# zrudnick/bramble

Hardware: AMD Instinct MI355X
Metric: projected alignments/sec vs GENCODE-scale annotation (higher is better)
Workload: dtype u32; 1 GPU; device-resident (inputs already in HBM, packed rows left in HBM): 10M paired-end 2x100 short reads (name-collated, unstranded) vs GENCODE-shaped synthetic annotation (250836 transcripts, 1684128 transcript-exon rows, 25 refs); BASELINE.json configs[1]; group_lanes=8, seed=0xb4a3b1e

## Files before the change

### bramble_amd/csrc/direct_kernels.inc

```

#define WAVE_SYNC()                                                \
  do {                                                             \
    __builtin_amdgcn_fence(__ATOMIC_RELEASE, "workgroup");         \
    __builtin_amdgcn_wave_barrier();                               \
    __builtin_amdgcn_fence(__ATOMIC_ACQUIRE, "workgroup");         \
  } while (0)

__global__ void __launch_bounds__(256) k_name_seed(DirectArgs D) {
  const int64_t g = (int64_t)blockIdx.x * blockDim.x + threadIdx.x;
  if (g >= D.n_groups) return;
  const uint32_t a0 = D.group_off[g];
  const uint32_t no = D.name_off[a0];
  Mt64Lazy gen;
  gen.seed(hash_bytes(D.names + no, D.name_off[a0 + 1] - no));
  D.rnd0[g] = gen();
}
__device__ __forceinline__ uint32_t pick_from(uint64_t z0, const uint8_t *name, uint64_t len, uint32_t n) {
  uint64_t hi, lo;
  mul64wide(z0, (uint64_t)n, hi, lo);
  if (lo < (uint64_t)n) {
    const uint64_t thr = (0 - (uint64_t)n) % (uint64_t)n;
    if (lo < thr) return primary_pick(name, len, n);
  }
  return (uint32_t)hi;
// ... 586 lines not shown
#pragma unroll
      for (int st = 32; st; st >>= 1) if (sh_pre[wv][l + st] <= e) l += st;
      D.m_aln[first + e] = sh_v[wv][l];
    }
  }
}

template <int CLS>
__global__ void __launch_bounds__(256, CLS == 1 ? 8 : 6) k_emit_rows(ProjectArgs A, DirectArgs D, int64_t first, int64_t n_end) {
  __shared__ uint32_t sh_cig[CLS == 1 ? 1 : 256 * LDS_SLOT];
  __shared__ uint16_t sh_mops[CLS == 1 ? 1 : 256];
  if (CLS != 1) {
    sh_mops[threadIdx.x] = (uint16_t)((merge_action(threadIdx.x >> 4, threadIdx.x & 15u) << 8) | merge_ops(threadIdx.x >> 4, threadIdx.x & 15u));
    __syncthreads();
  }
  const int64_t e64 = first + (int64_t)blockIdx.x * blockDim.x + threadIdx.x;
  if (e64 >= n_end) return;
  const DevIndex &ix = A.ix;
  const DevCfg &cfg = A.cfg;
  typedef uint32_t ntl4 __attribute__((ext_vector_type(4)));
  typedef uint32_t ntl2 __attribute__((ext_vector_type(2)));
  const uint32_t a = __builtin_nontemporal_load(D.m_aln + e64);
  if (a == 0xffffffffu) return;
  const ntl4 hd_ = __builtin_nontemporal_load((const ntl4 *)(A.head + a)), rg_ = __builtin_nontemporal_load((const ntl4 *)(A.ranges + a));
  const ntl2 f_ = __builtin_nontemporal_load((const ntl2 *)(D.fm + a)), gd_ = __builtin_nontemporal_load((const ntl2 *)(D.gd + a)), dp_ = __builtin_nontemporal_load((const ntl2 *)(D.dpos + a));
  const uint4 hd = make_uint4(hd_.x, hd_.y, hd_.z, hd_.w), rg = make_uint4(rg_.x, rg_.y, rg_.z, rg_.w);
  const uint2 f = make_uint2(f_.x, f_.y), gd = make_uint2(gd_.x, gd_.y), dp = make_uint2(dp_.x, dp_.y);
  const uint4 E = make_uint4(gd.x, gd.y, dp.x, dp.y);
  const uint32_t is_fast = CLS == 1;
  uint4 hd2 = make_uint4(0, 0, 0, 0);
  uint32_t c0 = 0, c1 = 0;
  RealCig rc;
  if (CLS != 1) { hd2 = A.head2[a]; c0 = A.cigar_off[a]; c1 = A.cigar_off[a + 1]; }
  const uint32_t n_seg = hd.z, rid = hd.w >> 2;
  const uint2 q0 = make_uint2(hd.x, hd.y);
  const int st0 = (n_seg == 1) ? ST_ONLY : ST_FIRST;
  const uint32_t n0 = rg.y - rg.x;
  if (CLS != 1) rc.fetch(A.cigar + c0, c1 - c0);
  const uint32_t k = (uint32_t)e64 - E.w;
  const uint64_t fmask = (uint64_t)f.x | ((uint64_t)f.y << 32);
  uint64_t mm = fmask;
  for (uint32_t j = 0; j < k; j++) mm &= mm - 1;
  const uint32_t item = (uint32_t)(__ffsll((long long)mm) - 1);
  const int s = item < n0 ? 0 : 1;
  const uint32_t row = s == 0 ? rg.x + item : rg.z + (item - n0);
  const uint4 r_a = ix.s_row[2 * (size_t)row], r_b = ix.s_row[2 * (size_t)row + 1];
  const uint32_t gs = r_a.x, gend = r_a.y;
  const uint4 pay = make_uint4(r_b.x, r_b.y, r_a.w, r_b.z);
  uint32_t c = 0;
  {
    for (uint64_t m2 = fmask; m2;) {
      uint32_t t8[8]; bool ok[8];
#pragma unroll
      for (int u = 0; u < 8; u++) {
        ok[u] = m2 != 0;
        const uint32_t b = ok[u] ? (uint32_t)(__ffsll((long long)m2) - 1) : item;
        m2 &= m2 - 1;
        t8[u] = ix.s_tid[b < n0 ? rg.x + b : rg.z + (b - n0)];
      }
#pragma unroll
      for (int u = 0; u < 8; u++) c += (ok[u] && t8[u] < pay.x) ? 1u : 0u;
    }
  }
  Hit h0;
  classify(s == 1, st0, q0.x, q0.y, gs, gend, pay.z, cfg, h0);
  if (is_fast) {
    const uint32_t os = q0.x > gs ? q0.x : gs, oe = q0.y < gend ? q0.y : gend;
    const uint32_t ml = oe - os;
    uint32_t w0, w1 = 0, w2 = 0, n_out;
    if (h0.left_ins) { w0 = CIG_GEN(h0.left_ins, OP_S); w1 = CIG_GEN(ml, OP_M); n_out = 2; if (h0.right_ins) { w2 = CIG_GEN(h0.right_ins, OP_S); n_out = 3; } }
    else { w0 = CIG_GEN(ml, OP_M); n_out = 1; if (h0.right_ins) { w1 = CIG_GEN(h0.right_ins, OP_S); n_out = 2; } }
    const uint32_t junc = ((h0.left_ins == 0 && h0.left_gap == 0) ? 1u : 0u) + ((h0.right_ins == 0 && h0.right_gap == 0) ? 1u : 0u);
    uint64_t cref = (uint64_t)w0 | ((uint64_t)w1 << 32);
    if (n_out == 3) {
      cref = D.cig_base[a] + (uint64_t)c * (1u + 2u * 6u);
      uint32_t *slot = A.cig_arena + cref;
      slot[0] = w0; slot[1] = w1; slot[2] = w2;
    }
    write_row(D, E, a, c, pay.x, h0.pos, n_out, s == 1, cref, junc, ml);
    return;
  }
  if (CLS == 1) return;
  ReadCtx rd;
  rd.n_seg = n_seg; rd.seg = A.seg + (size_t)c0 + (size_t)a; rd.real = A.cigar + c0; rd.n_real = c1 - c0; rd.q12 = hd2;
  const uint4 *Ex = ix.tx_ex + pay.w;
  const uint32_t i0 = pay.y & 0x7fffffffu;
  CandOut p1;
  bool plain = false;
  const uint32_t sb = ix.slab_off[2 * rid + s], se = ix.slab_off[2 * rid + s + 1];
  if (n_seg == 1) { p1.alive = true; p1.fwpos = h0.pos; p1.rcpos = h0.pos; p1.n_seg = 1; p1.n_gex = 1; p1.i_lastm = i0; p1.last_right_ins = h0.right_ins; p1.last_right_gap = h0.right_gap; }
  else if (!cfg.long_reads && !cfg.ignore_small_exons) {
    plain = true;
    p1.alive = true; p1.fwpos = h0.pos; p1.rcpos = h0.pos; p1.n_seg = n_seg; p1.n_gex = n_seg; p1.i_lastm = i0;
    p1.last_right_ins = 0; p1.last_right_gap = 0;
  }
  else p1 = walk_pass1(ix, cfg, rd, Ex, s == 1, sb, se, i0, make_uint4(gs, gend, pay.z, 0), make_uint2(r_a.z, r_b.w), q0, h0);
  const uint32_t ideal_cap = 4u * n_seg + 2u;
  const uint32_t cap = rd.n_real + 2u * ideal_cap;
  const uint64_t slot_off = D.cig_base[a] + (uint64_t)c * cap;
  uint32_t *slot = A.cig_arena + slot_off;
  uint32_t *lds = &sh_cig[(CLS == 1 ? 0 : threadIdx.x) * LDS_SLOT];
  const bool ideal_lds = ideal_cap <= LDS_IDEAL;
  uint32_t *ideal = ideal_lds ? lds : slot + rd.n_real + ideal_cap;
  Acc acc; IdealSink sk;
  sk.init(ideal);
  walk_pass2(ix, cfg, rd, Ex, s == 1, sb, se, i0, q0, make_uint4(gs, gend, pay.z, 0), make_uint2(r_a.z, r_b.w), h0, p1, acc, sk, no_clip(), no_clip());
  const uint32_t n_ideal = sk.finish();
  const bool out_lds = ideal_lds && (rd.n_real + n_ideal <= LDS_SLOT - LDS_IDEAL);
  uint32_t *outp = out_lds ? lds + LDS_IDEAL : slot;
  const uint32_t n_out = merge_cigars(rc, rd.n_real, ideal, n_ideal, outp, sh_mops);
  uint64_t cig_ref = slot_off;
  if (n_out <= 2) cig_ref = (uint64_t)(n_out > 0 ? outp[0] : 0u) | ((uint64_t)(n_out > 1 ? outp[1] : 0u) << 32);
// ... 43 lines not shown
```

### bramble_amd/csrc/kernels.h

```cpp
#pragma once
#include <hip/hip_runtime.h>
#include <stdint.h>

#include "device_types.h"
#include "ksw_types.h"

namespace br {

struct ProjectArgs {
  DevIndex ix;
  DevCfg cfg;
  int64_t n_aln;
  const int32_t *ref_id;
  const uint32_t *cigar_off;
  const uint32_t *cigar;
  const uint2 *seg;
  const AlnMeta *meta;
  const uint4 *head;
  const uint4 *head2;
  const uint32_t *fast_flag;
  const uint32_t *fast_pre;
  uint32_t *n_matches;
  uint4 *ranges;
  uint64_t *mask;
// ... 1 lines not shown
  uint32_t *n_big;
  uint32_t *walk_list;
  uint32_t *n_walk;
  uint32_t *m_aln;
  const uint32_t *match_off;
  const uint64_t *cig_base;
  uint32_t *m_tid, *m_aux;
  uint2 *m_p;
  uint2 *m_x;
  uint4 *m_b;
  uint64_t *m_cigoff;
  uint32_t *cig_arena;
  const uint64_t *tot;
  uint64_t lim_m, lim_c;
  uint64_t cover;
};
__device__ __forceinline__ bool tot_over(const uint64_t *tot, uint64_t lim_m, uint64_t lim_c) { return tot && (tot[0] > lim_m || tot[1] > lim_c); }

struct CountArgs {
  const uint32_t *slab_off, *bin_off, *s_start, *s_pmax;
  const uint4 *t_bin, *s_row, *tx_ex;
  uint32_t n_refs, bin_shift;
  uint32_t max_clip, max_junc_ins, max_junc_gap, max_error_exon;
  int32_t ignore_small_exons, long_reads;
  uint32_t n_aln;
  const uint4 *head, *head2;
  const uint32_t *cigar_off;
  const uint2 *seg;
  uint32_t *n_matches;
  uint64_t *mask;
  uint4 *ranges;
  uint32_t *walk_list, *n_walk;
  uint32_t *big_list, *n_big;
};

struct FaArgs {
  const int32_t *seq_src;
  const uint32_t *seq_off;
  const uint8_t *seqs;
  uint32_t *n_prob;
  uint32_t *seq_bytes;
  const uint32_t *prob_off;
  const uint64_t *seqarena_off;
  KswProb *probs;
  FaSrc *srcs;
  KswRes *results;
  uint8_t *seq_arena;
  uint32_t *clip_ops;
  uint32_t *ideal_cap;
  uint64_t *want_l, *want_r;
};

struct KswArgs {
  int64_t n_prob;
  const KswProb *probs;
  KswRes *results;
  const uint8_t *seq_arena;
  uint32_t *clip_ops;
  uint8_t *scratch;
  size_t scratch_per_wave, pmat_bytes, raw_words;
  int64_t n_waves;
  uint32_t tmax;
  uint64_t *stats;
  uint32_t *raw_out, *raw_n; int32_t *max_out; uint32_t raw_cap;
  const uint32_t *list; const uint32_t *n_list;
};
// ... 322 lines not shown
```

### bramble_amd/csrc/pipeline.cpp

```cpp
#include <algorithm>
#include <cstring>
#include <vector>

#include "ctx.h"

int ensure_aux_stream(br_ctx *c) {
  if (c->ksw_stream) return BR_OK;
  HIPCHK(hipStreamCreateWithPriority(&c->ksw_stream, hipStreamNonBlocking, 0));
  for (auto &e : c->ksw_ev) HIPCHK(hipEventCreateWithFlags(&e, hipEventDisableTiming));
  for (auto &e : c->aux_ev) HIPCHK(hipEventCreateWithFlags(&e, hipEventDisableTiming));
  return BR_OK;
}

int run_ksw(br_ctx *c, hipStream_t st, const KswRun &R) {
  if (R.n_prob <= 0) return BR_OK;
  const uint64_t n_all = (uint64_t)R.n_prob;
  const uint64_t qmax = std::max<uint64_t>(R.qmax, 1), tmax = std::max<uint64_t>(R.tmax, 1);
  KswArgs K{};
  K.n_prob = R.n_prob; K.probs = R.probs; K.results = R.results; K.seq_arena = R.seq_arena; K.clip_ops = R.clip_ops;
  K.stats = R.stats;
  K.raw_out = R.raw_out; K.raw_n = R.raw_n; K.max_out = R.max_out; K.raw_cap = R.raw_cap;
  auto general = [&](uint64_t n_work, uint64_t q_hi, uint64_t t_hi, const uint32_t *list, const uint32_t *n_list) -> int {
    q_hi = std::max<uint64_t>(q_hi, 1); t_hi = std::max<uint64_t>(t_hi, 1);
    K.tmax = (uint32_t)t_hi;
// ... 89 lines not shown

static int ensure_count_tables(br_ctx *c, const br_device_batch *b) {
  const int64_t n = b->n_aln;
  RC(c->seg.ensure((size_t)(b->n_cigar_words + n) * sizeof(uint2)));
  RC(c->meta.ensure((size_t)n * sizeof(AlnMeta))); RC(c->head.ensure((size_t)n * sizeof(uint4))); RC(c->head2.ensure((size_t)n * sizeof(uint4)));
  RC(c->fast_flag.ensure((size_t)n * 4)); RC(c->ranges.ensure((size_t)n * sizeof(uint4))); RC(c->mask.ensure((size_t)n * 8));
  RC(c->cig_base.ensure((size_t)(n + 1) * 8)); RC(c->big_list.ensure((size_t)n * 4)); RC(c->totals.ensure(16 * 8));
  return BR_OK;
}

static ProjectArgs count_args(br_ctx *c, const DevCfg &dc, const br_device_batch *b) {
  ProjectArgs A{};
  A.ix = c->ix->dev; A.cfg = dc; A.n_aln = b->n_aln; A.ref_id = b->ref_id; A.cigar_off = b->cigar_off; A.cigar = b->cigar;
  A.seg = c->seg.as<uint2>(); A.meta = c->meta.as<AlnMeta>(); A.head = c->head.as<uint4>(); A.head2 = c->head2.as<uint4>();
  A.fast_flag = c->fast_flag.as<uint32_t>(); A.n_matches = c->n_matches.as<uint32_t>();
  A.ranges = c->ranges.as<uint4>(); A.mask = c->mask.as<uint64_t>(); A.big_list = c->big_list.as<uint32_t>();
  return A;
}

static CountArgs count_view(const ProjectArgs &A) {
  CountArgs C{};
  const DevIndex &ix = A.ix;
  C.slab_off = ix.slab_off; C.bin_off = ix.bin_off; C.s_start = ix.s_start; C.s_pmax = ix.s_pmax;
  C.t_bin = ix.t_bin; C.s_row = ix.s_row; C.tx_ex = ix.tx_ex; C.n_refs = ix.n_refs; C.bin_shift = ix.bin_shift;
  C.max_clip = A.cfg.max_clip; C.max_junc_ins = A.cfg.max_junc_ins; C.max_junc_gap = A.cfg.max_junc_gap;
  C.max_error_exon = A.cfg.max_error_exon; C.ignore_small_exons = A.cfg.ignore_small_exons; C.long_reads = A.cfg.long_reads;
  C.n_aln = (uint32_t)A.n_aln;
  C.head = A.head; C.head2 = A.head2; C.cigar_off = A.cigar_off; C.seg = A.seg;
  C.n_matches = A.n_matches; C.mask = A.mask; C.ranges = A.ranges;
  C.walk_list = A.walk_list; C.n_walk = A.n_walk; C.big_list = A.big_list; C.n_big = A.n_big;
  return C;
}

static int count_pass(br_ctx *c, hipStream_t st, const ProjectArgs &A, Prof &pf, bool split) {
  const int n_blocks = c->n_cu * c->blocks_per_cu;
  if (!split || A.ix.n_rows == 0) {
    RC(pf.begin(BR_K_COUNT));
    launch_project(st, A, false, c->group_lanes, n_blocks);
    RC(pf.end());
    return BR_OK;
  }
  const CountArgs C = count_view(A);
  RC(pf.begin(BR_K_COUNT));
  launch_count(st, C, c->group_lanes, n_blocks, 1);
  RC(pf.end());
  RC(pf.begin(BR_K_COUNT_WALK));
  launch_count(st, C, c->group_lanes, n_blocks, 2);
  RC(pf.end());
  return BR_OK;
}

static int emit_match_table(hipStream_t st, const ProjectArgs &A, Prof &pf, int64_t n_list, int64_t n_simple) {
  if (!A.cfg.filter_by_similarity) {
    RC(pf.begin(BR_K_EMIT_SIMPLE));
    launch_emit_dense(st, A, n_list, n_simple, 1);
    RC(pf.end());
    RC(pf.begin(BR_K_EMIT));
    launch_emit_dense(st, A, n_list, n_simple, 2);
    RC(pf.end());
  } else {
    RC(pf.begin(BR_K_EMIT));
    launch_emit_dense(st, A, n_list, -1, 0);
    RC(pf.end());
  }
  return BR_OK;
}

static void finish_call(br_ctx *c, const DevCfg &dc, const br_device_batch *b, br_device_rows *out, uint64_t n_matches,
                        uint64_t n_rows, uint64_t n_pool, bool aux_cols) {
  out->n_matches = (int64_t)n_matches; out->n_rows = (int64_t)n_rows; out->n_pool_words = (int64_t)n_pool;
  out->total_complete = n_rows; out->total_unique = c->h_totals[5]; out->dropped_reads = c->h_totals[6];
  out->pool = c->cig_arena.as<uint32_t>(); out->row_off = c->row_off.as<uint64_t>();
  c->counters[6] = n_matches;
  c->last_n_rows = (int64_t)n_rows; c->last_n_aln = b->n_aln; c->last_n_pool = (int64_t)n_pool;
  c->last_aux_cols = aux_cols; c->wide_valid = false; c->detail_valid = false; c->last_l_qseq = b->l_qseq; c->last_long_reads = dc.long_reads;
// ... 175 lines not shown
  if (c->d_side_cap == 0) c->d_side_cap = std::max<uint64_t>((uint64_t)n / 4, 1u << 20);
  RC(c->d_side.ensure((size_t)c->d_side_cap * sizeof(uint2)));
  if (c->rows_busy_set && c->row_off.cap < (size_t)(n + 1) * 8) HIPCHK(hipEventSynchronize(c->rows_busy));
  RC(c->row_off.ensure((size_t)(n + 1) * 8));
  RC(ensure_aux_stream(c));
  hipStream_t ax = c->ksw_stream;
  uint64_t *d_tot = c->totals.as<uint64_t>();

  ProjectArgs A = count_args(c, dc, b);
  A.n_big = dz_nbig; A.walk_list = c->walk_list.as<uint32_t>(); A.n_walk = dz_nbig + 1;
  const bool have_names = b->names && b->name_off;
  DirectArgs D{};
  D.n_aln = n; D.n_groups = ng; D.group_off = b->group_off; D.aln_group = c->aln_group.as<uint32_t>(); D.mate_idx = b->mate_idx;
  D.n_matches = c->n_matches.as<uint32_t>(); D.mask = c->mask.as<uint64_t>(); D.ranges = c->ranges.as<uint4>();
  D.fast_flag = c->fast_flag.as<uint32_t>(); D.s_tid = ix->dev.s_tid; D.big_list = A.big_list; D.n_big = A.n_big;
  D.fm = c->d_fm.as<uint2>(); D.pm_list = (uint32_t *)(c->d_fm.as<uint2>() + n); D.pm_n = dz_nbig + 2; D.n_kept = c->d_nkept.as<uint32_t>(); D.n_rows = c->n_rows.as<uint32_t>(); D.pflag = c->pbit.as<uint8_t>();
  D.side = c->d_side.as<uint2>(); D.side_cap = c->d_side_cap; D.side_used = (unsigned long long *)(dz + GD_COUNTER_WORDS);
  D.cls_pos = c->d_clspos.as<uint32_t>(); D.cig_base = c->cig_base.as<uint64_t>(); D.row_off = c->row_off.as<uint64_t>();
  D.name_off = have_names ? b->name_off : nullptr; D.names = have_names ? b->names : nullptr; D.rnd0 = c->d_rnd.as<uint64_t>();
  D.gd = c->d_desc.as<uint2>(); D.dpos = c->d_desc.as<uint2>() + n; D.hi0 = c->d_hi0.as<uint32_t>(); D.counters = c->counters_d.as<uint64_t>(); D.tot = d_tot;

  if (!c->aux2_stream) { HIPCHK(hipStreamCreateWithPriority(&c->aux2_stream, hipStreamNonBlocking, 0)); HIPCHK(hipEventCreateWithFlags(&c->aux2_ev, hipEventDisableTiming)); }
  hipStream_t ax2 = c->aux2_stream;
  HIPCHK(hipMemsetAsync(dz, 0, (GD_COUNTER_WORDS + 4) * 8, st));
  HIPCHK(hipEventRecord(c->aux_ev[0], st));
  HIPCHK(hipStreamWaitEvent(ax, c->aux_ev[0], 0));
  RC(pf.begin(BR_K_SEGMENT));
  launch_segment(st, n, b->ref_id, b->ref_start, b->flags, b->xs, b->ts, b->cigar_off, b->cigar, dc, ix->n_refs,
                 c->seg.as<uint2>(), c->meta.as<AlnMeta>(), c->head.as<uint4>(), c->head2.as<uint4>(), c->fast_flag.as<uint32_t>());
  RC(pf.end());
  RC(pf.begin(BR_K_GROUP_IDS));
  launch_group_ids(st, ng, b->group_off, c->aln_group.as<uint32_t>());
  RC(pf.end());
  RC(count_pass(c, st, A, pf, true));
  if (c->rows_busy_set) { HIPCHK(hipStreamWaitEvent(st, c->rows_busy, 0)); }
  const int big_blocks = c->n_cu * 4;
  uint64_t kept = 0, arena = 0, n_simple = 0, n_rows = 0, n_raw = 0;
  bool expanded_ahead = false;
  if (have_names) {
    HIPCHK(hipEventRecord(c->aux_ev[7], st));
    HIPCHK(hipStreamWaitEvent(ax2, c->aux_ev[7], 0));
    RC(pf.begin(BR_K_NAME_SEED, ax2));
    launch_name_seed(ax2, D);
    RC(pf.end());
    HIPCHK(hipEventRecord(c->aux2_ev, ax2));
  }
  for (int attempt = 0;; attempt++) {
    if (attempt) {
      HIPCHK(hipMemsetAsync(dz, 0, (GD_COUNTER_WORDS + 2) * 8, st));
      HIPCHK(hipMemsetAsync(D.pm_n, 0, 4, st));
    }
    HIPCHK(hipEventRecord(c->aux_ev[1], st));
    HIPCHK(hipStreamWaitEvent(ax, c->aux_ev[1], 0));
    RC(pf.begin(BR_K_PAIR_BIG, ax));
    launch_big_collect(ax, A, D, big_blocks);
    launch_pair_big(ax, D, big_blocks);
    RC(pf.end());
    HIPCHK(hipEventRecord(c->aux_ev[2], ax));
    RC(pf.begin(BR_K_PAIR_MASK));
    launch_pair_mask(st, D, c->n_cu * 2);
    RC(pf.end());
    HIPCHK(hipStreamWaitEvent(st, c->aux_ev[2], 0));
    HIPCHK(hipEventRecord(c->aux_ev[3], st));
    HIPCHK(hipStreamWaitEvent(ax, c->aux_ev[3], 0));
    if (have_names) HIPCHK(hipStreamWaitEvent(ax, c->aux2_ev, 0));
    RC(pf.begin(BR_K_GROUP_DESC, ax));
    launch_group_desc(ax, D);
// ... 418 lines not shown
    RC(run_match_table(c, dc, b, st, &tmp, pf, false));
  }
  RC(c->totals.ensure(16 * 8));
  DevBuf stats; RC(stats.ensure(8 * 8));
  HIPCHK(hipMemsetAsync(stats.p, 0, 8 * 8, st));
  StatsArgs T{};
  T.ix = c->ix->dev; T.n_aln = b->n_aln; T.ref_id = b->ref_id; T.cigar_off = b->cigar_off;
  T.seg = c->seg.as<uint2>(); T.head = c->head.as<uint4>(); T.head2 = c->head2.as<uint4>(); T.out = stats.as<uint64_t>();
  int64_t nm = (int64_t)c->counters[6];
  launch_stats(st, T, nm ? c->m_p.as<uint2>() : nullptr, c->match_off.as<uint32_t>(), c->n_matches.as<uint32_t>());
  uint64_t h[8];
  HIPCHK(hipMemcpyAsync(h, stats.p, 8 * 8, hipMemcpyDeviceToHost, st));
  HIPCHK(hipStreamSynchronize(st));
  uint64_t n = (uint64_t)b->n_aln;
  c->counters[3] = h[3]; c->counters[4] = h[4]; c->counters[5] = h[5]; c->counters[7] = h[7];
  c->counters[0] = 24ull * n + 4ull * h[3];
  c->counters[1] = h[1];
  c->counters[2] = 4ull * n + 24ull * (uint64_t)nm + 4ull * h[7];
  return BR_OK;
}

extern "C" int br_ctx_direct_diag(br_ctx *c, uint64_t out[8], uint8_t *pflags) {
  if (!c || !out || !c->last_direct) return BR_ERR_INVALID_ARG;
  HIPCHK(hipSetDevice(c->ix->device));
  const DirectArgs &D = c->dD;
  uint64_t used = 0;
  uint32_t nb[3] = {0, 0, 0};
  HIPCHK(hipDeviceSynchronize());
  HIPCHK(hipMemcpy(&used, D.side_used, 8, hipMemcpyDeviceToHost));
  HIPCHK(hipMemcpy(nb, D.n_big, 12, hipMemcpyDeviceToHost));
  if (pflags && D.n_aln > 0) HIPCHK(hipMemcpy(pflags, D.pflag, (size_t)D.n_aln, hipMemcpyDeviceToHost));
  memset(out, 0, 8 * sizeof(uint64_t));
  out[0] = nb[0]; out[1] = (uint64_t)c->d_side_attempts; out[2] = used; out[3] = D.side_cap; out[4] = nb[2];
  return BR_OK;
}

extern "C" int br_project_batch_device(br_ctx *c, const br_config *cfg, const br_device_batch *b, void *stream,
                                       br_device_rows *out) {
  if (!c || !cfg || !b || !out) return BR_ERR_INVALID_ARG;
  return run_device(c, cfg, b, (hipStream_t)stream, out);
}

extern "C" int br_device_rows_expand(br_ctx *c, void *stream, br_device_wide_rows *out) {
  if (!c || !out) return BR_ERR_INVALID_ARG;
  return expand_rows(c, (hipStream_t)stream, out);
}
```

### bramble_amd/csrc/project_kernels.hip

```cpp
#include <hip/hip_runtime.h>
#include <stdint.h>

#include <algorithm>

#include "device_types.h"
#include "kernels.h"
#include "primary_pick.h"

namespace br {

#define CIG_OP(c) ((c) & 0xfu)
#define CIG_LEN(c) ((c) >> 4)
#define CIG_GEN(l, o) (((l) << 4) | (o))

__global__ void __launch_bounds__(256) k_segment(int64_t n_aln, const int32_t *__restrict__ ref_id,
                                                 const int32_t *__restrict__ ref_start,
                                                 const uint16_t *__restrict__ flags,
                                                 const int8_t *__restrict__ xs, const int8_t *__restrict__ ts,
                                                 const uint32_t *__restrict__ cigar_off,
                                                 const uint32_t *__restrict__ cigar, DevCfg cfg,
                                                 uint32_t n_refs, uint2 *__restrict__ seg,
                                                 AlnMeta *__restrict__ meta, uint4 *__restrict__ head,
                                                 uint4 *__restrict__ head2, uint32_t *__restrict__ fast_flag, SegExtra X) {
  int64_t a = (int64_t)blockIdx.x * blockDim.x + threadIdx.x;
// ... 52 lines not shown
    char c = (char)xs[a];
    if (c == 0) {
      char m = (char)ts[a];
      if (m == '+' || m == '-') c = (f & 0x10) ? ((m == '+') ? '-' : '+') : m;
    }
    char strand = (c == '+' || c == '-') ? c : '.';
    if (strand == '.' && (cfg.fr || cfg.rf)) {
      bool is_rev = f & 0x10;
      bool cond = (cfg.rf && is_rev) || (cfg.fr && !is_rev);
      if (f & 0x1) {
        int order = (f & 0x40) ? 1 : ((f & 0x80) ? 2 : 0);
        strand = (order == 1) ? (cond ? '-' : '+') : (cond ? '+' : '-');
      } else {
        strand = cond ? '-' : '+';
      }
    }
    smode = (strand == '+') ? 1u : (strand == '-') ? 2u : 3u;
  }
  uint32_t lclip = 0, rclip = 0;
  if (cfg.long_reads) {
    if (n_cigar == 0) { n = 0; }
    else {
      uint32_t w0 = cg[0];
      if (CIG_OP(w0) == OP_H) { if (n_cigar > 1 && CIG_OP(cg[1]) == OP_S) lclip = CIG_LEN(cg[1]); }
      else if (CIG_OP(w0) == OP_S) lclip = CIG_LEN(w0);
      uint32_t wl = cg[n_cigar - 1];
      if (CIG_OP(wl) == OP_H) { if (n_cigar >= 2 && CIG_OP(cg[n_cigar - 2]) == OP_S) rclip = CIG_LEN(cg[n_cigar - 2]); }
      else if (CIG_OP(wl) == OP_S) rclip = CIG_LEN(wl);
    }
  }
  if (cfg.long_reads) { AlnMeta m; m.n_seg = n; m.smode = smode; m.n_left_clip = lclip; m.n_right_clip = rclip; meta[a] = m; }
  uint2 q0 = n ? e0 : make_uint2(0, 0);
  head[a] = make_uint4(q0.x, q0.y, n, n ? (((uint32_t)rid << 2) | smode) : 0u);
  if (n > 1) { const uint2 q2 = n > 2 ? e2 : make_uint2(0, 0); head2[a] = make_uint4(e1.x, e1.y, q2.x, q2.y); }
  uint32_t fast = (n == 1 && n_cigar == 1 && CIG_OP(cg[0]) == OP_M && !cfg.filter_by_similarity && !cfg.long_reads) ? 1u : 0u;
  fast_flag[a] = (fast << 31) | ((n_cigar + 2u * (4u * n + 2u)) & 0x7fffffffu);
}

struct Hit { uint32_t pos, left_ins, right_ins, left_gap, right_gap; };

__device__ __forceinline__ bool classify(bool minus, int status, uint32_t qs, uint32_t qe, uint32_t s,
                                         uint32_t e, uint32_t pos_start, const DevCfg &c, Hit &h) {
  const bool junc_left = (status == ST_MIDDLE || status == ST_LAST);
  const bool junc_right = (status == ST_FIRST || status == ST_MIDDLE);
  const uint32_t lg = qs > s ? qs - s : 0u, li = s > qs ? s - qs : 0u;
  const uint32_t rg = e > qe ? e - qe : 0u, ri = qe > e ? qe - e : 0u;
  const uint32_t lim_li = junc_left ? c.max_junc_ins : c.max_clip;
  const uint32_t lim_ri = (junc_right || minus) ? c.max_junc_ins : c.max_clip;
  const uint32_t lim_lg = junc_left ? c.max_junc_gap : 0xffffffffu;
  const uint32_t lim_rg = junc_right ? c.max_junc_gap : 0xffffffffu;
  h.pos = pos_start + (minus ? rg : lg); h.left_ins = li; h.right_ins = ri; h.left_gap = lg; h.right_gap = rg;
  return (li <= lim_li) & (ri <= lim_ri) & (lg <= lim_lg) & (rg <= lim_rg);
}

struct IdealSink {
  uint32_t *buf; uint32_t n; uint32_t cur; bool has;
  __device__ __forceinline__ void init(uint32_t *b) { buf = b; n = 0; cur = 0; has = false; }
  __device__ __forceinline__ void add(uint32_t len, uint32_t op) {
    const bool same = has && CIG_OP(cur) == op;
    const bool flush = has && !same;
    if (flush && buf) buf[n] = cur;
    n += flush ? 1u : 0u;
    cur = same ? cur + (len << 4) : CIG_GEN(len, op);
    has = true;
  }
  __device__ __forceinline__ uint32_t finish() { if (has) { if (buf) buf[n] = cur; n++; has = false; } return n; }
};
// ... 524 lines not shown
            bool in = r < rb[k];
            uint32_t v = in ? ((k & 1) ? ix.s_pmax[r] : ix.s_start[r]) : 0u;
            bool t = in && ((k & 1) ? (v <= q0.x) : (v < q0.y));
            res[k] += (uint32_t)__popcll((__ballot(t) >> gbase) & gmask);
          }
        }
        hi[0] = res[0]; lo[0] = res[1] < res[0] ? res[1] : res[0];
        hi[1] = res[2]; lo[1] = res[3] < res[2] ? res[3] : res[2];
      }
      if (gl == 0) A.ranges[a] = make_uint4(lo[0], hi[0], lo[1], hi[1]);
    }
    uint32_t n0 = hi[0] - lo[0], n1 = hi[1] - lo[1];
    uint32_t n_items = n0 + n1;

    ReadCtx rd;
    rd.n_seg = n_seg; rd.seg = nullptr; rd.real = nullptr; rd.n_real = 0; rd.q12 = hd2;
    uint32_t moff = 0; uint64_t cbase = 0; uint32_t cap = 0, ideal_cap = 0;
    bool have_mask = false; uint64_t mask_in = 0;
    if (EMIT || n_seg > 3) {
      uint32_t c0 = A.cigar_off[a];
      rd.seg = A.seg + (size_t)c0 + (size_t)a;
      if constexpr (EMIT) { rd.real = A.cigar + c0; rd.n_real = A.cigar_off[a + 1] - c0; }
    }
    if constexpr (EMIT) {
      moff = A.match_off[a]; cbase = A.cig_base[a];
      ideal_cap = 4u * n_seg + 2u;
      cap = rd.n_real + 2u * ideal_cap;
      have_mask = n_items <= 64;
      mask_in = have_mask ? A.mask[a] : 0;
    }
    uint32_t total = 0;
    uint64_t mask_all = 0;
    bool defer = false;

    const int n_sweeps = (EMIT && !have_mask) ? 2 : 1;
    uint32_t aux_n = 0;
    for (int sweep = 0; sweep < n_sweeps; sweep++) {
      for (uint32_t base = 0; base < n_items; base += G) {
        uint32_t item = base + (uint32_t)gl;
        bool valid = item < n_items;
        bool alive = false;
        int s = 0; uint32_t row = 0, gs = 0, gend = 0, nxt = 0, nxe = 0;
        uint4 pay = make_uint4(0xffffffffu, 0, 0, 0);
        Hit h0; CandOut p1; const uint4 *E = nullptr; uint32_t i0 = 0;
        p1.alive = false; p1.fwpos = 0; p1.rcpos = 0; p1.n_seg = 0; p1.n_gex = 0;
        h0.pos = 0; h0.left_ins = h0.right_ins = h0.left_gap = h0.right_gap = 0;
        if (valid) {
          s = item < n0 ? 0 : 1;
          row = s == 0 ? lo[0] + item : lo[1] + (item - n0);
          const uint4 r_a = ix.s_row[2 * (size_t)row], r_b = ix.s_row[2 * (size_t)row + 1];
          gs = r_a.x; gend = r_a.y; nxt = r_a.z; nxe = r_b.w; pay = make_uint4(r_b.x, r_b.y, r_a.w, r_b.z);
          bool want = true;
          if (EMIT && have_mask) want = (mask_in >> item) & 1ull;
          if (want && gend > q0.x && gs < q0.y && classify(s == 1, st0, q0.x, q0.y, gs, gend, pay.z, cfg, h0)) {
            E = ix.tx_ex + pay.w; i0 = pay.y & 0x7fffffffu;
            bool superseded = false;
            if (nxt < q0.y) {
              for (uint32_t i = i0 + 1;; i++) {
                uint4 e = E[i];
                if (e.x >= q0.y) break;
                Hit hx;
                if (e.y > q0.x && classify(s == 1, st0, q0.x, q0.y, e.x, e.y, e.z, cfg, hx)) { superseded = true; break; }
              }
            }
            if (!superseded) {
              if (n_seg == 1) { p1.alive = true; p1.fwpos = h0.pos; p1.rcpos = h0.pos; p1.n_seg = 1; p1.n_gex = 1; p1.i_lastm = i0; p1.last_right_ins = h0.right_ins; p1.last_right_gap = h0.right_gap; }
              else if (!EMIT && !SIMF && n_seg == 2 && (nxt >= hd2.y || nxe >= hd2.y)) {
                const uint32_t qs1 = hd2.x, qe1 = hd2.y;
                Hit hh;
                bool alive2 = false;
                if (gend < qe1 && !(qs1 == q0.x && qe1 == q0.y)) {
                  const bool c0 = gend > qs1 && classify(s == 1, ST_LAST, qs1, qe1, gs, gend, pay.z, cfg, hh);
                  const uint4 e1 = next_row(make_uint4(gs, gend, pay.z, 0), make_uint2(nxt, nxe), s == 1);
                  const bool c1 = nxt < qe1 && nxe > qs1 && classify(s == 1, ST_LAST, qs1, qe1, e1.x, e1.y, e1.z, cfg, hh);
                  alive2 = c1 && !c0;
                }
                p1.alive = alive2;
              }
              else if (MODE == 1 && !cfg.long_reads && !cfg.ignore_small_exons && !(pay.y >> 31)) {
                const uint32_t qs1 = hd2.x, qe1 = hd2.y;
                const int st1 = n_seg == 2 ? ST_LAST : ST_MIDDLE;
                Hit hh;
                if (gend < qe1 && !(qs1 == q0.x && qe1 == q0.y)) {
                  const bool c0 = gend > qs1 && classify(s == 1, st1, qs1, qe1, gs, gend, pay.z, cfg, hh);
                  const uint4 e1 = next_row(make_uint4(gs, gend, pay.z, 0), make_uint2(nxt, nxe), s == 1);
                  const bool c1 = nxt < qe1 && nxe > qs1 && classify(s == 1, st1, qs1, qe1, e1.x, e1.y, e1.z, cfg, hh);
                  if (c1 && !c0) defer = true;
                }
                p1.alive = false;
              }
              else if (MODE == 1) { defer = true; p1.alive = false; }
              else p1 = walk_pass1(ix, cfg, rd, E, s == 1, sb[s], se[s], i0, make_uint4(gs, gend, pay.z, 0), make_uint2(nxt, nxe), q0, h0);
              alive = p1.alive;
            }
          }
        }
        Acc acc; IdealSink sk; double score = 0.0;
        if (!EMIT || !have_mask) {
          if (SIMF && alive) {
            sk.init(nullptr);
            walk_pass2(ix, cfg, rd, E, s == 1, sb[s], se[s], i0, q0, make_uint4(gs, gend, pay.z, 0), make_uint2(nxt, nxe), h0, p1, acc, sk, no_clip(), no_clip());
            alive = similarity(cfg, acc, score);
          }
        }
        uint32_t rank = 0;
        bool do_emit = false;
        if constexpr (!EMIT) {
          uint64_t m = (__ballot(alive) >> gbase) & gmask;
          total += (uint32_t)__popcll(m);
          if (base < 64) mask_all |= (G == 64) ? m : (m << base);
        } else if (have_mask) {
          uint64_t mm = mask_in;
          while (mm) {
            int b = __ffsll((long long)mm) - 1; mm &= mm - 1;
            uint32_t t2;
            if ((uint32_t)b >= base && (uint32_t)b < base + G) t2 = __shfl(pay.x, b - (int)base, G);
            else {
              uint32_t r2 = (uint32_t)b < n0 ? lo[0] + (uint32_t)b : lo[1] + ((uint32_t)b - n0);
              t2 = ix.s_tid[r2];
            }
            rank += (t2 < pay.x) ? 1u : 0u;
          }
          do_emit = alive;
        } else {
          uint64_t m = (__ballot(alive) >> gbase) & gmask;
          if (sweep == 0) {
            if (alive) {
              uint32_t k = aux_n + (uint32_t)__popcll(m & ((1ull << gl) - 1ull));
              A.m_aux[moff + k] = pay.x;
// ... 12 lines not shown
          uint32_t *ideal = ideal_lds ? lds : slot + rd.n_real + ideal_cap;
          sk.init(ideal);
          walk_pass2(ix, cfg, rd, E, s == 1, sb[s], se[s], i0, q0, make_uint4(gs, gend, pay.z, 0), make_uint2(nxt, nxe), h0, p1, acc, sk, no_clip(), no_clip());
          uint32_t n_ideal = sk.finish();
          similarity(cfg, acc, score);
          bool out_lds = ideal_lds && (rd.n_real + n_ideal <= LDS_SLOT - LDS_IDEAL);
          uint32_t *outp = out_lds ? lds + LDS_IDEAL : slot;
          RealCig rc; rc.fetch(rd.real, rd.n_real);
          uint32_t n_out = merge_cigars(rc, rd.n_real, ideal, n_ideal, outp);
          uint64_t cig_ref = cbase + (uint64_t)rank * cap;
          if (n_out <= 2) cig_ref = (uint64_t)(n_out > 0 ? outp[0] : 0u) | ((uint64_t)(n_out > 1 ? outp[1] : 0u) << 32);
          else if (out_lds) for (uint32_t k = 0; k < n_out; k++) slot[k] = outp[k];
          uint32_t mi = moff + rank;
          A.m_tid[mi] = pay.x;
          A.m_p[mi] = make_uint2((s == 0) ? p1.fwpos : p1.rcpos, n_out | ((uint32_t)s << 31));
          A.m_x[mi] = make_uint2((uint32_t)acc.junc_hits, (uint32_t)acc.ref_consumed);
          if (SIMF) {
            unsigned long long sb64 = (unsigned long long)__double_as_longlong(score);
            A.m_b[mi] = make_uint4((uint32_t)acc.clip_score, 0u, (uint32_t)sb64, (uint32_t)(sb64 >> 32));
          }
          A.m_cigoff[mi] = cig_ref;
        }
      }
      if (EMIT && !have_mask && sweep == 0) __threadfence_block();
    }
    if (MODE == 1 && ((__ballot(defer) >> gbase) & gmask) != 0) {
      if (gl == 0) {
        uint32_t k = atomicAdd(&sh_wn, 1u);
        if (k < WALK_LDS) sh_wl[MODE == 1 ? k : 0] = (uint32_t)a;
        else { uint32_t k2 = atomicAdd(A.n_walk, 1u); A.walk_list[k2] = (uint32_t)a; }
      }
      continue;
    }
    if (!EMIT && gl == 0) {
      A.n_matches[a] = total; A.mask[a] = mask_all;
      if (n_items > 64 && total) {
        const uint32_t k = atomicAdd(&sh_bn, 1u);
        if (k < BIG_LDS) sh_bl[EMIT ? 0 : k] = (uint32_t)a;
        else { const uint32_t k2 = atomicAdd(A.n_big, 1u); A.big_list[k2] = (uint32_t)a; }
      }
    }
  }
  if (!EMIT) {
    __syncthreads();
    const uint32_t n_loc = sh_bn < BIG_LDS ? sh_bn : BIG_LDS;
    if (threadIdx.x == 0) sh_bbase = n_loc ? atomicAdd(A.n_big, n_loc) : 0u;
    __syncthreads();
    for (uint32_t i = threadIdx.x; i < n_loc; i += blockDim.x) A.big_list[sh_bbase + i] = sh_bl[EMIT ? 0 : i];
  }
  if (MODE == 1) {
    __syncthreads();
    const uint32_t n_loc = sh_wn < WALK_LDS ? sh_wn : WALK_LDS;
    if (threadIdx.x == 0) sh_wbase = n_loc ? atomicAdd(A.n_walk, n_loc) : 0u;
    __syncthreads();
    for (uint32_t i = threadIdx.x; i < n_loc; i += blockDim.x) A.walk_list[sh_wbase + i] = sh_wl[MODE == 1 ? i : 0];
  }
}

__device__ __forceinline__ void expand_chunk(const ProjectArgs &A, int64_t a, uint32_t (*sh_pre)[64], uint32_t (*sh_v)[64]) {
  const int lane = threadIdx.x & 63, wv = threadIdx.x >> 6;
  uint32_t nm = 0, pos = 0, v = 0;
  bool fast = false;
  if (a < A.n_aln) nm = A.n_matches[a];
  if (nm) {
    const uint32_t fp = A.fast_pre[a];
    fast = A.fast_flag[a] >> 31;
    pos = fast ? fp : A.fast_pre[A.n_aln] + (A.match_off[a] - fp);
    const uint4 rg = A.ranges[a];
// ... 1115 lines not shown
```

### bramble_amd/lib.py

```python
import ctypes as C
import os

import numpy as np

_HERE = os.path.dirname(os.path.abspath(__file__))
LIB_PATH = os.path.join(_HERE, "libbramble_amd.so")
_P = C.POINTER

K_SEGMENT, K_COUNT, K_EMIT, K_PAIR_COUNT, K_PAIR_EMIT, K_GATHER, K_SCAN, K_EMIT_AUX, K_KSW, K_BAM, K_PARSE, K_CODEC, K_EMIT_SIMPLE, K_PRIMARY, K_CIGAR_POOL, K_COUNT_WALK, K_EXPAND, K_GROUP_IDS, K_P1, K_P1_WALK, K_EMIT_WL, K_NAME_SEED, K_PAIR_MASK, K_PAIR_BIG, K_GROUP_DESC, K_EXPAND_ROWS, K_EMIT_ROWS_SIMPLE, K_EMIT_ROWS, K_BIG_EMIT, K_NUM = range(30)
KERNEL_NAMES = ["k_segment", "k_project<G,false,false,1>", "k_emit_dense<false,2>", "k_pair<false>", "k_pair<true>",
                "k_rows", "k_scan_*", "k_project<64,true>", "k_ksw", "k_bam_scan+k_bam_size+k_bam_encode",
                "k_rec_fields+k_group_off+k_rec_copy+k_mates+k_seq_*", "k_deflate_*+k_bgzf_compact",
                "k_emit_dense<false,1>", "k_primary", "(unused)", "k_project<G,false,false,2>", "k_expand", "k_group_ids",
                "(unused)", "(unused)", "(unused)", "k_name_seed", "k_pair_mask", "k_big<0>+k_pair_big", "k_group_desc",
                "k_expand_rows", "k_emit_rows<1>", "k_emit_rows<2>", "k_big<1>"]


class BrambleError(RuntimeError):
    pass


class BrExon(C.Structure):
    _fields_ = [("start", C.c_uint32), ("end", C.c_uint32)]

# ... 504 lines not shown

    @staticmethod
    def _device_batch_struct(dev_batch):
        db = BrDeviceBatch()
        db.n_aln = dev_batch["n_aln"]
        db.n_groups = dev_batch["n_groups"]
        for name in ("ref_id", "ref_start", "flags", "xs", "ts", "cigar_off", "cigar", "mate_idx", "group_off",
                     "l_qseq"):
            setattr(db, name, dev_batch[name].data_ptr())
        db.n_cigar_words = dev_batch["n_cigar_words"]
        db.max_n_cigar = dev_batch["max_n_cigar"]
        if dev_batch.get("seqs") is not None:
            db.seq_off = dev_batch["seq_off"].data_ptr()
            db.seqs = dev_batch["seqs"].data_ptr()
            db.seq_src = dev_batch["seq_src"].data_ptr()
            db.max_soft_clip = dev_batch["max_soft_clip"]
        if dev_batch.get("names") is not None:
            db.name_off = dev_batch["name_off"].data_ptr()
            db.names = dev_batch["names"].data_ptr()
        return db

    def collect_counters(self, dev_batch, stream=0):
        db = self._device_batch_struct(dev_batch)
        check(lib().br_ctx_collect_counters(self.h, C.byref(db), C.c_void_p(stream)), "br_ctx_collect_counters")
        out = (C.c_uint64 * 8)()
        check(lib().br_ctx_last_counters(self.h, out), "br_ctx_last_counters")
        keys = ("B_in", "B_idx", "B_out", "n_cigar", "read_exons", "overlap_hits", "matches", "out_cigar_words")
        return dict(zip(keys, [int(v) for v in out]))

    def direct_diag(self, n_aln=None):
        out = (C.c_uint64 * 8)()
        pf = np.zeros(n_aln, dtype=np.uint8) if n_aln is not None else None
        check(lib().br_ctx_direct_diag(self.h, out, pf.ctypes.data if pf is not None and n_aln else None), "br_ctx_direct_diag")
        d = dict(zip(("n_big", "side_attempts", "side_used", "side_cap", "pm_n"), [int(v) for v in out[:5]]))
        if pf is not None:
            d["pflags"] = pf
        return d

    def project_bam_device(self, cfg, blob, rec_off, rec_len, ref_map, stream=0):
        recs = BrDeviceRecords()
        recs.blob = blob.data_ptr()
        recs.rec_off = rec_off.data_ptr()
        recs.n_aln = rec_len.numel()
        recs.rec_len = rec_len.data_ptr()
        rm = np.ascontiguousarray(ref_map, dtype=np.int32)
        rows, out = BrDeviceRows(), BrDeviceBam()
        check(lib().br_project_bam_device(self.h, C.byref(cfg), C.byref(recs), rm.ctypes.data, len(rm), C.c_void_p(stream),
                                          C.byref(rows), C.byref(out)), "br_project_bam_device")
        return rows, out

    def bgzf_deflate_device(self, src, stream=0):
        import torch
        from .device import _DevArray
        out, n = C.c_void_p(), C.c_uint64()
        check(lib().br_bgzf_deflate_device(self.h, C.c_void_p(src.data_ptr()), src.numel(), C.c_void_p(stream), C.byref(out),
                                           C.byref(n)), "br_bgzf_deflate_device")
        if n.value == 0:
            return torch.zeros(0, dtype=torch.uint8, device=src.device)
        return torch.as_tensor(_DevArray(out.value, n.value, "|u1"), device=src.device)

    def bgzf_inflate_device(self, src, blocks, stream=0):
        import torch
        from .device import _DevArray
        out, n = C.c_void_p(), C.c_uint64()
        blocks = np.ascontiguousarray(blocks, dtype=BGZF_BLOCK)
        L = lib()
        L.br_bgzf_inflate_device.argtypes = [C.c_void_p, C.c_void_p, C.c_uint64, C.c_void_p, C.c_int64, C.c_void_p, _P(C.c_void_p), _P(C.c_uint64)]
# ... 315 lines not shown
```

Before: 2.856 billion alignments/s.

## Route exact two-segment spliced reads through the fast emit path

The segment kernel marks two-segment M-N-M alignments in head2. During counting, alignments whose matches all hit exon boundaries exactly are flagged as 'light' by setting the fast bit in fast_flag. The fast emit path then projects the second segment inline with classify and next_row, skipping the full walk and cigar-building path. It also adds a diagnostic counter for light alignments. The risk is a mismatch in cigar arena slot sizing or junction counting compared with the general path.

```diff
diff --git a/bramble_amd/csrc/direct_kernels.inc b/bramble_amd/csrc/direct_kernels.inc
--- a/bramble_amd/csrc/direct_kernels.inc
+++ b/bramble_amd/csrc/direct_kernels.inc
@@ -642,6 +642,7 @@
   uint32_t c0 = 0, c1 = 0;
   RealCig rc;
   if (CLS != 1) { hd2 = A.head2[a]; c0 = A.cigar_off[a]; c1 = A.cigar_off[a + 1]; }
+  else if (hd.z == 2) hd2 = A.head2[a];
   const uint32_t n_seg = hd.z, rid = hd.w >> 2;
   const uint2 q0 = make_uint2(hd.x, hd.y);
   const int st0 = (n_seg == 1) ? ST_ONLY : ST_FIRST;
@@ -676,18 +677,29 @@
   classify(s == 1, st0, q0.x, q0.y, gs, gend, pay.z, cfg, h0);
   if (is_fast) {
     const uint32_t os = q0.x > gs ? q0.x : gs, oe = q0.y < gend ? q0.y : gend;
-    const uint32_t ml = oe - os;
+    uint32_t ml = oe - os, pos = h0.pos, r_ins = h0.right_ins, junc_in = 0;
+    bool r_exact = h0.right_ins == 0 && h0.right_gap == 0;
+    if (n_seg == 2) {
+      const uint2 q1 = make_uint2(hd2.x, hd2.y);
+      const uint4 e1 = next_row(make_uint4(gs, gend, pay.z, 0), make_uint2(r_a.z, r_b.w), s == 1);
+      Hit hh;
+      classify(s == 1, ST_LAST, q1.x, q1.y, e1.x, e1.y, e1.z, cfg, hh);
+      ml += (q1.y < e1.y ? q1.y : e1.y) - q1.x;
+      pos = s == 0 ? h0.pos : hh.pos;
+      r_ins = hh.right_ins; r_exact = hh.right_ins == 0 && hh.right_gap == 0;
+      junc_in = 2;
+    }
     uint32_t w0, w1 = 0, w2 = 0, n_out;
-    if (h0.left_ins) { w0 = CIG_GEN(h0.left_ins, OP_S); w1 = CIG_GEN(ml, OP_M); n_out = 2; if (h0.right_ins) { w2 = CIG_GEN(h0.right_ins, OP_S); n_out = 3; } }
-    else { w0 = CIG_GEN(ml, OP_M); n_out = 1; if (h0.right_ins) { w1 = CIG_GEN(h0.right_ins, OP_S); n_out = 2; } }
-    const uint32_t junc = ((h0.left_ins == 0 && h0.left_gap == 0) ? 1u : 0u) + ((h0.right_ins == 0 && h0.right_gap == 0) ? 1u : 0u);
+    if (h0.left_ins) { w0 = CIG_GEN(h0.left_ins, OP_S); w1 = CIG_GEN(ml, OP_M); n_out = 2; if (r_ins) { w2 = CIG_GEN(r_ins, OP_S); n_out = 3; } }
+    else { w0 = CIG_GEN(ml, OP_M); n_out = 1; if (r_ins) { w1 = CIG_GEN(r_ins, OP_S); n_out = 2; } }
+    const uint32_t junc = junc_in + ((h0.left_ins == 0 && h0.left_gap == 0) ? 1u : 0u) + (r_exact ? 1u : 0u);
     uint64_t cref = (uint64_t)w0 | ((uint64_t)w1 << 32);
     if (n_out == 3) {
-      cref = D.cig_base[a] + (uint64_t)c * (1u + 2u * 6u);
+      cref = D.cig_base[a] + (uint64_t)c * (n_seg == 2 ? 3u + 2u * 10u : 1u + 2u * 6u);
       uint32_t *slot = A.cig_arena + cref;
       slot[0] = w0; slot[1] = w1; slot[2] = w2;
     }
-    write_row(D, E, a, c, pay.x, h0.pos, n_out, s == 1, cref, junc, ml);
+    write_row(D, E, a, c, pay.x, pos, n_out, s == 1, cref, junc, ml);
     return;
   }
   if (CLS == 1) return;
diff --git a/bramble_amd/csrc/kernels.h b/bramble_amd/csrc/kernels.h
--- a/bramble_amd/csrc/kernels.h
+++ b/bramble_amd/csrc/kernels.h
@@ -57,6 +57,7 @@
   uint4 *ranges;
   uint32_t *walk_list, *n_walk;
   uint32_t *big_list, *n_big;
+  uint32_t *light_flag;
 };
 
 struct FaArgs {
diff --git a/bramble_amd/csrc/pipeline.cpp b/bramble_amd/csrc/pipeline.cpp
--- a/bramble_amd/csrc/pipeline.cpp
+++ b/bramble_amd/csrc/pipeline.cpp
@@ -145,7 +145,7 @@
   return C;
 }
 
-static int count_pass(br_ctx *c, hipStream_t st, const ProjectArgs &A, Prof &pf, bool split) {
+static int count_pass(br_ctx *c, hipStream_t st, const ProjectArgs &A, Prof &pf, bool split, bool light = false) {
   const int n_blocks = c->n_cu * c->blocks_per_cu;
   if (!split || A.ix.n_rows == 0) {
     RC(pf.begin(BR_K_COUNT));
@@ -153,7 +153,8 @@
     RC(pf.end());
     return BR_OK;
   }
-  const CountArgs C = count_view(A);
+  CountArgs C = count_view(A);
+  if (light) C.light_flag = const_cast<uint32_t *>(A.fast_flag);
   RC(pf.begin(BR_K_COUNT));
   launch_count(st, C, c->group_lanes, n_blocks, 1);
   RC(pf.end());
@@ -395,7 +396,7 @@
   RC(pf.begin(BR_K_GROUP_IDS));
   launch_group_ids(st, ng, b->group_off, c->aln_group.as<uint32_t>());
   RC(pf.end());
-  RC(count_pass(c, st, A, pf, true));
+  RC(count_pass(c, st, A, pf, true, true));
   if (c->rows_busy_set) { HIPCHK(hipStreamWaitEvent(st, c->rows_busy, 0)); }
   const int big_blocks = c->n_cu * 4;
   uint64_t kept = 0, arena = 0, n_simple = 0, n_rows = 0, n_raw = 0;
@@ -880,6 +881,20 @@
   if (pflags && D.n_aln > 0) HIPCHK(hipMemcpy(pflags, D.pflag, (size_t)D.n_aln, hipMemcpyDeviceToHost));
   memset(out, 0, 8 * sizeof(uint64_t));
   out[0] = nb[0]; out[1] = (uint64_t)c->d_side_attempts; out[2] = used; out[3] = D.side_cap; out[4] = nb[2];
+  if (D.n_aln > 0) {
+    const size_t n = (size_t)D.n_aln;
+    std::vector<uint32_t> ff(n), nk(n);
+    std::vector<uint4> hd(n);
+    std::vector<uint8_t> pf(n);
+    HIPCHK(hipMemcpy(ff.data(), D.fast_flag, n * 4, hipMemcpyDeviceToHost));
+    HIPCHK(hipMemcpy(nk.data(), D.n_kept, n * 4, hipMemcpyDeviceToHost));
+    HIPCHK(hipMemcpy(hd.data(), c->head.p, n * sizeof(uint4), hipMemcpyDeviceToHost));
+    HIPCHK(hipMemcpy(pf.data(), D.pflag, n, hipMemcpyDeviceToHost));
+    uint64_t light = 0;
+    for (size_t a = 0; a < n; a++)
+      if ((ff[a] >> 31) && hd[a].z == 2 && !(pf[a] & PF_BIG)) light += nk[a];
+    out[5] = light;
+  }
   return BR_OK;
 }
 
diff --git a/bramble_amd/csrc/project_kernels.hip b/bramble_amd/csrc/project_kernels.hip
--- a/bramble_amd/csrc/project_kernels.hip
+++ b/bramble_amd/csrc/project_kernels.hip
@@ -108,7 +108,12 @@
   if (cfg.long_reads) { AlnMeta m; m.n_seg = n; m.smode = smode; m.n_left_clip = lclip; m.n_right_clip = rclip; meta[a] = m; }
   uint2 q0 = n ? e0 : make_uint2(0, 0);
   head[a] = make_uint4(q0.x, q0.y, n, n ? (((uint32_t)rid << 2) | smode) : 0u);
-  if (n > 1) { const uint2 q2 = n > 2 ? e2 : make_uint2(0, 0); head2[a] = make_uint4(e1.x, e1.y, q2.x, q2.y); }
+  if (n > 1) {
+    const bool mnm = n == 2 && n_cigar == 3 && pre4 && CIG_OP(w4[0]) == OP_M && CIG_OP(w4[2]) == OP_M && !cfg.filter_by_similarity &&
+                     !cfg.long_reads && !cfg.ignore_small_exons;
+    const uint2 q2 = n > 2 ? e2 : make_uint2(mnm ? 1u : 0u, 0);
+    head2[a] = make_uint4(e1.x, e1.y, q2.x, q2.y);
+  }
   uint32_t fast = (n == 1 && n_cigar == 1 && CIG_OP(cg[0]) == OP_M && !cfg.filter_by_similarity && !cfg.long_reads) ? 1u : 0u;
   fast_flag[a] = (fast << 31) | ((n_cigar + 2u * (4u * n + 2u)) & 0x7fffffffu);
 }
@@ -699,6 +704,7 @@
     uint32_t total = 0;
     uint64_t mask_all = 0;
     bool defer = false;
+    uint32_t inexact = 0;
 
     const int n_sweeps = (EMIT && !have_mask) ? 2 : 1;
     uint32_t aux_n = 0;
@@ -762,6 +768,7 @@
             }
           }
         }
+        if (MODE == 1 && PRE == 1) inexact += (alive && (gend != q0.y || nxt != hd2.x)) ? 1u : 0u;
         Acc acc; IdealSink sk; double score = 0.0;
         if (!EMIT || !have_mask) {
           if (SIMF && alive) {
@@ -840,8 +847,12 @@
       }
       continue;
     }
+    bool light = false;
+    if constexpr (MODE == 1 && CNT && PRE == 1)
+      light = n_seg == 2 && hd2.z != 0 && n_items <= 64 && ((__ballot(inexact != 0u) >> gbase) & gmask) == 0;
     if (!EMIT && gl == 0) {
       A.n_matches[a] = total; A.mask[a] = mask_all;
+      if constexpr (MODE == 1 && CNT && PRE == 1) { if (light && A.light_flag) A.light_flag[a] = (1u << 31) | (3u + 2u * (4u * 2u + 2u)); }
       if (n_items > 64 && total) {
         const uint32_t k = atomicAdd(&sh_bn, 1u);
         if (k < BIG_LDS) sh_bl[EMIT ? 0 : k] = (uint32_t)a;
diff --git a/bramble_amd/lib.py b/bramble_amd/lib.py
--- a/bramble_amd/lib.py
+++ b/bramble_amd/lib.py
@@ -560,7 +560,7 @@
         out = (C.c_uint64 * 8)()
         pf = np.zeros(n_aln, dtype=np.uint8) if n_aln is not None else None
         check(lib().br_ctx_direct_diag(self.h, out, pf.ctypes.data if pf is not None and n_aln else None), "br_ctx_direct_diag")
-        d = dict(zip(("n_big", "side_attempts", "side_used", "side_cap", "pm_n"), [int(v) for v in out[:5]]))
+        d = dict(zip(("n_big", "side_attempts", "side_used", "side_cap", "pm_n", "light"), [int(v) for v in out[:6]]))
         if pf is not None:
             d["pflags"] = pf
         return d
```

Measured after the change: 3.014 billion alignments/s (median of 6 runs). +5.5%, better.
